# dendisuhubdy/neural_sound_generation

Hardware: AMD Instinct MI355X
Metric: mel-frames/sec VQ-VAE fwd+bwd+Adam (80-mel x 1024) (higher is better)
Workload: dtype bf16; 1 GPU; BASELINE configs[1]: VQVAE(1,dim=128,z_dim=512) train step, 128 clips/GPU x 80-mel x 1024 frames; clips_per_gpu=128, global_batch=128, frames=1024, parallelism=dp1

## Files before the change

neural_sound_generation_amd/csrc/gemm_patch.hip:

```cpp
#include "nsg_common.h"
#include <type_traits>

namespace {

NSG_DIAG_SWITCH(int, g_patch_gemm, 1)
NSG_DIAG_SWITCH(int, g_patch_grid_cap, 512)


inline int patch_grid(int ntiles, int ntn)
{
    const int cap = g_patch_grid_cap > 0 ? (g_patch_grid_cap / ntn > 0 ? g_patch_grid_cap / ntn : 1) : 0;
    return (cap > 0 && ntiles > cap) ? cap : ntiles;
}

constexpr int PG_MAX_JOBS = 16;
constexpr int PG_MAX_TAPS = 64;
constexpr int SLOT_BYTES = 16;

struct PatchJob {
    int c0_bytes;
    short jy, jx;
    short oy, ox;
    int flush;
};
struct PatchTap {
    int delta_bytes;
    unsigned woff_bytes;
};

struct PatchGemmParams {
    const bf16_t *in;
    const bf16_t *w;
    const float *bias;
    bf16_t *out;
    const bf16_t *epi_add;
    const bf16_t *epi_mask;
    int B, IH, IW, CI, OH, OW, CO;
    int tiles_y, tiles_x, ntiles;
    FastDiv div_tx, div_tyx;
    int njobs, ntaps;
    int sy, sx;
    int os;
    int flags;
    unsigned in_bytes, w_bytes;
    unsigned long long *stamps;
    float *stats;
    PatchJob jobs[PG_MAX_JOBS];
    PatchTap taps[PG_MAX_TAPS];
};

template <int PH, int PW, int NT, bool ADD, bool MASK, bool STAMP = false, bool STATS = false>
__global__ __launch_bounds__(256) __attribute__((amdgpu_waves_per_eu(2))) void patch_gemm_kernel(const PatchGemmParams p)
{
    constexpr bool PRIV = !(ADD || MASK);
    constexpr int NSLOT = PH * PW;
    constexpr int NPIECE = NSLOT * 8;
    constexpr int NP = (NPIECE + 255) / 256;
    constexpr int NB = (NT == 9) ? 3 : 4;
    constexpr int LD = (NT == 9) ? 3 : 2;
    static_assert(NT % NB == 0 && NB % LD == 0 && NB >= 2, "static buffer roles inside a body of NB taps");
    constexpr int NLOAD = NT - LD;
    constexpr int PPT = (NP + NLOAD - 1) / NLOAD;
    constexpr int NSLOT_PAD = (NSLOT + 15) / 16 * 16;
    constexpr int PLANE = NSLOT_PAD * 16;
    constexpr int BUF_BYTES = 8 * PLANE;
    constexpr int CPITCH = 132;
    static_assert(32 * CPITCH * 4 <= BUF_BYTES, "a tile row of the output must fit a retired patch buffer");
    static_assert(PPT * NLOAD >= NP && NT >= 4, "every patch piece is fetched LD taps before the job ends");
    constexpr unsigned OOB = 0xfffffff0u;

    constexpr int STG_PITCH = 36;
    constexpr int STG_BYTES = 32 * STG_PITCH * 4;

    extern __shared__ __attribute__((aligned(16))) char smem[];

    unsigned long long st_entry = 0, st_rt = 0, st_loop = 0, st_bound = 0, st_flush = 0, st_pro = 0, st_jobs = 0, st_t = 0;
    auto now = [&]() -> unsigned long long {
        if constexpr (STAMP) {
            unsigned long long t;
            __builtin_amdgcn_sched_barrier(0);
            asm volatile("s_memtime %0\n\ts_waitcnt lgkmcnt(0)" : "=s"(t) :: "memory");
            __builtin_amdgcn_sched_barrier(0);
            return t;
        }
        return 0ull;
    };
    if constexpr (STAMP) { st_entry = now(); st_rt = __builtin_amdgcn_s_memrealtime(); }

    const int tid = threadIdx.x;
    const int lane = tid & 63;
    const int wave = __builtin_amdgcn_readfirstlane(tid >> 6);
    const int x31 = lane & 31, h = lane >> 5;
    const int n0 = blockIdx.y * 128;

    const __amdgpu_buffer_rsrc_t rs_in = __builtin_amdgcn_make_buffer_rsrc(const_cast<bf16_t *>(p.in), 0, (int)p.in_bytes, 0x00020000);
    const __amdgpu_buffer_rsrc_t rs_w = __builtin_amdgcn_make_buffer_rsrc(const_cast<bf16_t *>(p.w), 0, (int)p.w_bytes, 0x00020000);

    const int slot0 = (tid & 7) + 8 * (tid >> 6);
    const unsigned piece_b = ((tid >> 3) & 7) * 16;
    const unsigned pc_lds0 = ((tid >> 3) & 7) * PLANE + slot0 * 16;

    const unsigned wlane = (unsigned)((((n0 >> 5) + wave) * 4 * 64 + lane) * 16);
    unsigned arow[4];
#pragma unroll
    for (int y = 0; y < 4; ++y) arow[y] = (unsigned)((y * PW + x31) * 16 + h * PLANE);

    const int cg = tid & 15;
    const int ep = lane >> 2, eq = lane & 3;
    const int ech = PRIV ? 32 * wave + 8 * eq : 8 * cg;
    float bv[8];
#pragma unroll
    for (int e = 0; e < 8; ++e) bv[e] = p.bias ? p.bias[n0 + ech + e] : 0.f;
    const bool relu_out = (p.flags & NSG_RELU_OUT) != 0;
    static_assert(!STATS || (PRIV && !ADD && !MASK), "statistics ride in the plain variant's wave-private epilogue");
    float st_sum[STATS ? 8 : 1], st_sq[STATS ? 8 : 1], st_pv[STATS ? 8 : 1], st_cnt = 0.f;
#pragma unroll
    for (int e = 0; e < (STATS ? 8 : 1); ++e) { st_sum[e] = 0.f; st_sq[e] = 0.f; st_pv[e] = 0.f; }

    const int tab_delta = p.taps[lane].delta_bytes;
    const int tab_woff = (int)p.taps[lane].woff_bytes;
    static_assert(PG_MAX_TAPS <= 64, "one lane per table entry");
    auto tap_delta = [&](int q) { return __builtin_amdgcn_readlane(tab_delta, q); };
    auto tap_woff = [&](int q) { return __builtin_amdgcn_readlane(tab_woff, q); };
    const PatchJob myjob = p.jobs[lane & (PG_MAX_JOBS - 1)];
    const int tabj_c0 = myjob.c0_bytes;
    const int tabj_j = ((int)myjob.jy & 0xffff) | ((int)myjob.jx << 16);
    const int tabj_o = (int)myjob.oy | ((int)myjob.ox << 8) | (myjob.flush << 16);
    auto job_entry = [&](int j) {
        const int c0 = __builtin_amdgcn_readlane(tabj_c0, j), jj = __builtin_amdgcn_readlane(tabj_j, j), oo = __builtin_amdgcn_readlane(tabj_o, j);
        return PatchJob{c0, (short)(jj & 0xffff), (short)(jj >> 16), (short)(oo & 0xff), (short)((oo >> 8) & 0xff), (oo >> 16) & 1};
    };

    v16f acc[4];
    v4f breg[NB][4];
    v4f afr[4];
    v4f ptmp[LD][PPT];

    const int G = gridDim.x;
    struct Cursor { int tile, job; };
    auto advance = [&](Cursor &c) {
        if (++c.job == p.njobs) { c.job = 0; c.tile += G; }
    };
    auto tile_origin = [&](int tile, int &b, int &ty, int &tx) {
        b = nsg_div(tile, p.div_tyx);
        const int rem = tile - b * (p.tiles_y * p.tiles_x);
        ty = nsg_div(rem, p.div_tx);
        tx = rem - ty * p.tiles_x;
    };

    int pt_ok = 0, pt_iy0 = 0, pt_ix0 = 0;
    unsigned pt_base = 0;
    auto patch_origin = [&](const Cursor &c) {
        pt_ok = c.tile < p.ntiles;
        int b, ty, tx;
        tile_origin(pt_ok ? c.tile : 0, b, ty, tx);
        const PatchJob jb = job_entry(c.job);
        pt_iy0 = ty * 4 * p.sy + jb.jy;
        pt_ix0 = tx * 32 * p.sx + jb.jx;
        pt_base = (unsigned)(b * p.IH * p.IW) * (unsigned)p.CI * 2u + (unsigned)jb.c0_bytes;
    };
    auto load_piece = [&](int r) -> v4f {
        const int slot = slot0 + 32 * r;
        const int yy = slot / PW, xx = slot - yy * PW;
        const int iy = pt_iy0 + yy * p.sy, ix = pt_ix0 + xx * p.sx;
        const bool ok = (slot < NSLOT) & (iy >= 0) & (iy < p.IH) & (ix >= 0) & (ix < p.IW) & (pt_ok != 0);
        const unsigned off = ok ? pt_base + (unsigned)((iy * p.IW + ix) * p.CI) * 2u + piece_b : OOB;
        return __builtin_bit_cast(v4f, __builtin_amdgcn_raw_buffer_load_b128(rs_in, (int)off, 0, 0));
    };
    auto store_piece = [&](int buf, int r, const v4f v) {
        if (slot0 + 32 * r < NSLOT) *reinterpret_cast<v4f *>(smem + buf * BUF_BYTES + pc_lds0 + r * 32 * 16) = v;
    };
    auto patch_traffic = [&](auto HALF, int t, int buf) __attribute__((always_inline)) {
        constexpr int hf = decltype(HALF)::value;
        if (t >= LD) {
#pragma unroll
            for (int i = 0; i < PPT; ++i)
                if ((t - LD) * PPT + i < NP) store_piece(buf ^ 1, (t - LD) * PPT + i, ptmp[hf][i]);
        }
        if (t < NLOAD) {
#pragma unroll
            for (int i = 0; i < PPT; ++i)
                if (t * PPT + i < NP) ptmp[hf][i] = load_piece(t * PPT + i);
        }
    };

    auto load_b = [&](v4f (&bq)[4], int q) {
        const int so = tap_woff(q);
#if defined(NSG_DIAG) && defined(NSG_PATCH_FAKEW)
        bq[0] = __builtin_bit_cast(v4f, __builtin_amdgcn_raw_buffer_load_b128(rs_w, (int)wlane, so, 0));
        bq[1] = bq[0]; bq[2] = bq[0]; bq[3] = bq[0];
        return;
#endif
#pragma unroll
        for (int kk = 0; kk < 4; ++kk)
            bq[kk] = __builtin_bit_cast(v4f, __builtin_amdgcn_raw_buffer_load_b128(rs_w, (int)(wlane + 1024 * kk), so, 0));
    };
    auto read_a = [&](int y, int buf, int q, int kk) {
        afr[y] = *reinterpret_cast<const v4f *>(smem + buf * BUF_BYTES + tap_delta(q) + 2 * kk * PLANE + arow[y]);
    };
    auto read_a_first = [&](int buf, int q) {
#pragma unroll
        for (int y = 0; y < 4; ++y) read_a(y, buf, q, 0);
    };
    auto mfma_chain = [&](const v4f (&bq)[4], int buf, int q, int qn) __attribute__((always_inline)) {
#pragma unroll
        for (int kk = 0; kk < 4; ++kk) {
#pragma unroll
            for (int y = 0; y < 4; ++y) {
                acc[y] = __builtin_amdgcn_mfma_f32_32x32x16_bf16(__builtin_bit_cast(bf16x8, bq[kk]), __builtin_bit_cast(bf16x8, afr[y]), acc[y], 0, 0, 0);
                if (kk < 3) read_a(y, buf, q, kk + 1);
                else read_a(y, buf, qn, 0);
            }
#pragma unroll
            for (int y = 0; y < 4; ++y) {
                __builtin_amdgcn_sched_group_barrier(0x008, 1, 0);
                __builtin_amdgcn_sched_group_barrier(0x100, 1, 0);
            }
        }
    };
    const unsigned out_bytes = (unsigned)(p.B * p.OH * p.OW) * (unsigned)p.CO * 2u;
    const __amdgpu_buffer_rsrc_t rs_out = __builtin_amdgcn_make_buffer_rsrc(p.out, 0, (int)out_bytes, 0x00020000);
    const __amdgpu_buffer_rsrc_t rs_add = __builtin_amdgcn_make_buffer_rsrc(const_cast<bf16_t *>(ADD ? p.epi_add : p.out), 0, (int)out_bytes, 0x00020000);
    const __amdgpu_buffer_rsrc_t rs_mask = __builtin_amdgcn_make_buffer_rsrc(const_cast<bf16_t *>(MASK ? p.epi_mask : p.out), 0, (int)out_bytes, 0x00020000);
    unsigned eoff[4][2];
    v4f addv[ADD ? 4 : 1][2], maskv[MASK ? 4 : 1][2];
    auto epi_offsets = [&](int tile, const PatchJob &jb, bool live) {
        int b, ty, tx;
        tile_origin(tile, b, ty, tx);
#pragma unroll
        for (int y = 0; y < 4; ++y)
#pragma unroll
            for (int e2 = 0; e2 < 2; ++e2) {
                const int oy = (ty * 4 + y) * p.os + jb.oy;
                const int ox = (tx * 32 + (PRIV ? ep : (tid >> 4)) + 16 * e2) * p.os + jb.ox;
                eoff[y][e2] = (live && oy < p.OH && ox < p.OW) ? (unsigned)(((b * p.OH + oy) * p.OW + ox) * p.CO + n0 + ech) * 2u : OOB;
            }
    };
    auto epi_prefetch = [&]() {
        if constexpr (ADD) {
#pragma unroll
            for (int y = 0; y < 4; ++y)
#pragma unroll
                for (int e2 = 0; e2 < 2; ++e2) addv[y][e2] = __builtin_bit_cast(v4f, __builtin_amdgcn_raw_buffer_load_b128(rs_add, (int)eoff[y][e2], 0, 0));
        }
        if constexpr (MASK) {
#pragma unroll
            for (int y = 0; y < 4; ++y)
#pragma unroll
                for (int e2 = 0; e2 < 2; ++e2) maskv[y][e2] = __builtin_bit_cast(v4f, __builtin_amdgcn_raw_buffer_load_b128(rs_mask, (int)eoff[y][e2], 0, 0));
        }
    };
    auto tap = [&](auto JJ, int buf, int t, int q, int qn, int qb) __attribute__((always_inline)) {
        constexpr int J = decltype(JJ)::value;
        const v4f (&bq)[4] = breg[J];
        load_b(breg[(J + NB - 1) % NB], qb);
        __builtin_amdgcn_sched_barrier(0);
        patch_traffic(std::integral_constant<int, J % LD>{}, t, buf);
        __builtin_amdgcn_sched_barrier(0);
        mfma_chain(bq, buf, q, qn);
    };
    auto zero_acc = [&]() {
#pragma unroll
        for (int y = 0; y < 4; ++y)
#pragma unroll
            for (int r = 0; r < 16; ++r) acc[y][r] = 0.f;
    };

    auto epi_piece = [&](const v4f t0, const v4f t1, int y, int e2) __attribute__((always_inline)) {
        float v[8] = {t0.x, t0.y, t0.z, t0.w, t1.x, t1.y, t1.z, t1.w};
#pragma unroll
        for (int e = 0; e < 8; ++e) v[e] += bv[e];
#pragma unroll
        for (int e = 0; e < 8; ++e) v[e] = relu_out ? fmaxf(v[e], 0.f) : v[e];
        if constexpr (ADD) {
            float t[8];
            Elem<bf16_t>::unpack16(addv[y][e2], t);
#pragma unroll
            for (int e = 0; e < 8; ++e) v[e] += t[e];
        }
        if constexpr (MASK) {
            float t[8];
            Elem<bf16_t>::unpack16(maskv[y][e2], t);
#pragma unroll
            for (int e = 0; e < 8; ++e) v[e] = t[e] > 0.f ? v[e] : 0.f;
        }
        unsigned u[4];
#pragma unroll
        for (int i = 0; i < 4; ++i) u[i] = nsg_pack_bf16(v[2 * i], v[2 * i + 1]);
        if constexpr (STATS) {
            const float live = eoff[y][e2] != OOB ? 1.f : 0.f;
#pragma unroll
            for (int i = 0; i < 4; ++i) {
                const float y0 = nsg_bitsf(u[i] << 16), y1 = nsg_bitsf(u[i] & 0xffff0000u);
                st_pv[2 * i] = (st_cnt == 0.f) ? y0 : st_pv[2 * i];
                st_pv[2 * i + 1] = (st_cnt == 0.f) ? y1 : st_pv[2 * i + 1];
                const float d0 = (y0 - st_pv[2 * i]) * live, d1 = (y1 - st_pv[2 * i + 1]) * live;
                st_sum[2 * i] += d0;
                st_sum[2 * i + 1] += d1;
                st_sq[2 * i] = __builtin_fmaf(d0, d0, st_sq[2 * i]);
                st_sq[2 * i + 1] = __builtin_fmaf(d1, d1, st_sq[2 * i + 1]);
            }
            st_cnt += live;
        }
        typedef unsigned u4 __attribute__((ext_vector_type(4)));
        __builtin_amdgcn_raw_buffer_store_b128(u4{u[0], u[1], u[2], u[3]}, rs_out, (int)eoff[y][e2], 0, 0);
    };
    auto flush = [&](int tile, const PatchJob &jb, int buf) __attribute__((always_inline)) {
        if constexpr (PRIV) {
            epi_offsets(tile, jb, true);
            float *Sw = reinterpret_cast<float *>(smem + 2 * BUF_BYTES + wave * STG_BYTES);
            float *wdst = Sw + x31 * STG_PITCH + 4 * h;
            const float *rsrc = Sw + ep * STG_PITCH + 8 * eq;
            auto put_row = [&](int y) {
#pragma unroll
                for (int g = 0; g < 4; ++g)
                    *reinterpret_cast<v4f *>(wdst + 8 * g) = v4f{acc[y][4 * g], acc[y][4 * g + 1], acc[y][4 * g + 2], acc[y][4 * g + 3]};
                __builtin_amdgcn_wave_barrier();
            };
            v4f rd[2][2][2];
            auto get_row = [&](int y) {
#pragma unroll
                for (int e2 = 0; e2 < 2; ++e2) {
                    rd[y & 1][e2][0] = *reinterpret_cast<const v4f *>(rsrc + 16 * e2 * STG_PITCH);
                    rd[y & 1][e2][1] = *reinterpret_cast<const v4f *>(rsrc + 16 * e2 * STG_PITCH + 4);
                }
                __builtin_amdgcn_wave_barrier();
            };
            put_row(0);
            get_row(0);
#pragma unroll
            for (int y = 0; y < 4; ++y) {
                if (y < 3) { put_row(y + 1); get_row(y + 1); }
#pragma unroll
                for (int e2 = 0; e2 < 2; ++e2) epi_piece(rd[y & 1][e2][0], rd[y & 1][e2][1], y, e2);
            }
            return;
        }
        epi_offsets(tile, jb, true);
        epi_prefetch();
        float *Cs = reinterpret_cast<float *>(smem + buf * BUF_BYTES);
#pragma unroll
        for (int y = 0; y < 4; ++y) {
#pragma unroll
            for (int g = 0; g < 4; ++g) {
                float *dst = Cs + x31 * CPITCH + 32 * wave + 8 * g + 4 * h;
                *reinterpret_cast<v4f *>(dst) = v4f{acc[y][4 * g], acc[y][4 * g + 1], acc[y][4 * g + 2], acc[y][4 * g + 3]};
            }
            __syncthreads();
#pragma unroll
            for (int e2 = 0; e2 < 2; ++e2) {
                const int px = (tid >> 4) + 16 * e2;
                epi_piece(*reinterpret_cast<const v4f *>(Cs + px * CPITCH + 8 * cg), *reinterpret_cast<const v4f *>(Cs + px * CPITCH + 8 * cg + 4), y, e2);
            }
            __syncthreads();
        }
    };

    int bid = blockIdx.x;
    {
        const int xcd = bid & 7, qq = G >> 3, rr = G & 7;
        bid = (xcd < rr ? xcd * (qq + 1) : rr * (qq + 1) + (xcd - rr) * qq) + (bid >> 3);
    }
    Cursor cur = {bid, 0};
    Cursor pre = cur;
    if (cur.tile >= p.ntiles) return;
    patch_origin(pre);
    for (int r = 0; r < NP; ++r) store_piece(0, r, load_piece(r));
#pragma unroll
    for (int j = 0; j + 1 < NB; ++j) load_b(breg[j], j);
    zero_acc();
    __syncthreads();
    int buf = 0;
    auto run_job = [&](int qbase, int qnext_base) __attribute__((always_inline)) {
        using NO = std::integral_constant<bool, false>;
        using YES = std::integral_constant<bool, true>;
        auto tq = [&](int t) { return t < NT ? qbase + t : qnext_base + (t - NT); };
        auto body = [&](int t0, auto LASTBODY) __attribute__((always_inline)) {
            constexpr bool LB = decltype(LASTBODY)::value;
#define NSG_TAP(J)                                                                                                              \
            if constexpr (J < NB) {                                                                                             \
                constexpr int NEXT = (LB && J == NB - 1) ? 0 : 1;                                                               \
                tap(std::integral_constant<int, J>{}, buf, t0 + J, qbase + t0 + J, qbase + t0 + J + NEXT, tq(t0 + J + NB - 1)); \
            }
            NSG_TAP(0) NSG_TAP(1) NSG_TAP(2) NSG_TAP(3)
#undef NSG_TAP
        };
        read_a_first(buf, qbase);
#pragma unroll 1
        for (int t0 = 0; t0 < NT - NB; t0 += NB) body(t0, NO{});
        body(NT - NB, YES{});
    };
    if constexpr (STAMP) st_pro = now() - st_entry;
    auto do_job = [&]() __attribute__((always_inline)) {
        if constexpr (STAMP) st_t = now();
        const PatchJob jb = job_entry(cur.job);
        advance(pre);
        patch_origin(pre);
        const int qbase = cur.job * NT;
        const int qnext = (cur.job + 1 == p.njobs ? 0 : cur.job + 1) * NT;
        run_job(qbase, qnext);
        if constexpr (STAMP) { const unsigned long long t = now(); st_loop += t - st_t; st_t = t; st_jobs += 1; }
        __syncthreads();
        if constexpr (STAMP) { const unsigned long long t = now(); st_bound += t - st_t; st_t = t; }
        if (jb.flush) {
            flush(cur.tile, jb, buf);
            zero_acc();
            if constexpr (STAMP) { const unsigned long long t = now(); st_flush += t - st_t; st_t = t; }
        }
        advance(cur);
        buf ^= 1;
    };
    for (;;) {
        if (cur.tile >= p.ntiles) break;
        do_job();
    }
    if constexpr (STATS) {
        __syncthreads();
        float *red = reinterpret_cast<float *>(smem);
        const float inv = st_cnt > 0.f ? 1.f / st_cnt : 0.f;
#pragma unroll
        for (int e = 0; e < 8; ++e) {
            red[e * 256 + tid] = st_pv[e] + st_sum[e] * inv;
            red[(8 + e) * 256 + tid] = fmaxf(st_sq[e] - st_sum[e] * st_sum[e] * inv, 0.f);
        }
        red[16 * 256 + tid] = st_cnt;
        __syncthreads();
        if (tid < 128) {
            const int ch = tid, wv = ch >> 5, eqq = (ch >> 3) & 3, e = ch & 7;
            double N = 0.0, S = 0.0;
            for (int r = 0; r < 16; ++r) {
                const int t = wv * 64 + r * 4 + eqq;
                const double n = red[16 * 256 + t];
                N += n;
                S += n * (double)red[e * 256 + t];
            }
            const double mu = N > 0.0 ? S / N : 0.0;
            double Q = 0.0;
            for (int r = 0; r < 16; ++r) {
                const int t = wv * 64 + r * 4 + eqq;
                const double n = red[16 * 256 + t];
                const double dl = (double)red[e * 256 + t] - mu;
                Q += n > 0.0 ? (double)red[(8 + e) * 256 + t] + n * dl * dl : 0.0;
            }
            float *dst = p.stats + (size_t)blockIdx.x * 3 * p.CO + n0 + ch;
            dst[0] = (float)N;
            dst[p.CO] = (float)S;
            dst[2 * p.CO] = (float)Q;
        }
    }
    if constexpr (STAMP) {
        if (tid == 0 && p.stamps) {
            unsigned long long *o = p.stamps + 8 * (size_t)(blockIdx.y * gridDim.x + blockIdx.x);
            o[0] = now() - st_entry; o[1] = __builtin_amdgcn_s_memrealtime() - st_rt; o[2] = st_loop; o[3] = st_bound;
            o[4] = st_flush; o[5] = st_pro; o[6] = st_jobs;
#ifdef NSG_PATCH_ABS_STAMPS
            o[3] = st_rt; o[5] = __builtin_amdgcn_s_memrealtime();
#endif
            o[7] = ((unsigned long long)__builtin_amdgcn_s_getreg(6164) << 32) | (unsigned)__builtin_amdgcn_s_getreg(63492);
        }
    }
}

template <int PH, int PW, int NT, bool ADD, bool MASK, bool STAMP, bool STATS = false>
int launch_patch(const PatchGemmParams &p, int ntiles_n, hipStream_t s)
{
    constexpr int NSLOT = PH * PW;
    constexpr size_t BUF_BYTES = (size_t)8 * ((NSLOT + 15) / 16 * 16) * 16;
    constexpr bool PRIV = !(ADD || MASK);
    const size_t lds = 2 * BUF_BYTES + (PRIV ? 4 * 32 * 36 * 4 : 0);
    static LdsOptIn once;
    if (lds > 65536) {
        const int rc = nsg_lds_opt_in(once, {reinterpret_cast<const void *>(&patch_gemm_kernel<PH, PW, NT, ADD, MASK, STAMP, STATS>)}, lds, "patch_gemm");
        if (rc != NSG_OK) return rc;
    }
    const int gx = patch_grid(p.ntiles, ntiles_n);
    hipLaunchKernelGGL((patch_gemm_kernel<PH, PW, NT, ADD, MASK, STAMP, STATS>), dim3((unsigned)gx, (unsigned)ntiles_n), dim3(256), lds, s, p);
    return nsg_check_launch("patch_gemm");
}

template <int PH, int PW, int NT, bool STAMP>
int launch_patch_epi(const PatchGemmParams &p, int ntiles_n, hipStream_t s)
{
    if constexpr (!STAMP) {
        if (p.stats) return launch_patch<PH, PW, NT, false, false, false, true>(p, ntiles_n, s);
    }
    if (p.epi_add && p.epi_mask) return launch_patch<PH, PW, NT, true, true, STAMP>(p, ntiles_n, s);
    if (p.epi_add) return launch_patch<PH, PW, NT, true, false, STAMP>(p, ntiles_n, s);
    if (p.epi_mask) return launch_patch<PH, PW, NT, false, true, STAMP>(p, ntiles_n, s);
    return launch_patch<PH, PW, NT, false, false, STAMP>(p, ntiles_n, s);
}


}

#ifdef NSG_DIAG
extern "C" NSG_API void nsg_debug_set_patch_gemm(int on) { g_patch_gemm = on; }
extern "C" NSG_API void nsg_debug_set_patch_grid(int cap) { g_patch_grid_cap = cap; }
#endif

static int patch_kind(const GatherGemmParams &g)
{
    if (!g_patch_gemm) return -1;
    if (g.in_dtype != NSG_BF16 || g.out_dtype != NSG_BF16) return -1;
    if (g.flags & (NSG_RELU_IN | NSG_TANH_OUT)) return -1;
    if (g.stats && (g.epi_add || g.epi_mask || (g.flags & NSG_RELU_OUT) || g.stamps)) return -1;
    if (g.CI % 64 != 0 || g.CO % 128 != 0) return -1;
    const int chunks = g.CI / 64;
    int kind;
    if (g.mode == 1) kind = 2;
    else if (g.KH == 3 && g.KW == 3 && g.stride == 1 && g.pad >= 0 && g.pad <= 2 && g.pad_w >= 0 && g.pad_w <= 2) kind = 0;
    else if (g.KH == 4 && g.KW == 4 && g.stride == 2 && g.pad == 1 && g.pad_w == 1) kind = 1;
    else return -1;
    const int njobs = kind == 0 ? chunks : 4 * chunks;
    const int ntaps = kind == 0 ? 9 : 4;
    if (njobs > PG_MAX_JOBS || njobs * ntaps > PG_MAX_TAPS) return -1;
    if ((int64_t)g.B * nsg_cdiv(g.RH, 4) * nsg_cdiv(g.RW, 32) > 0x3fffffff) return -1;
    return kind;
}

int nsg_patch_gemm_stat_records(const GatherGemmParams &g)
{
    if (patch_kind(g) < 0) return 0;
    return patch_grid((int)((int64_t)g.B * nsg_cdiv(g.RH, 4) * nsg_cdiv(g.RW, 32)), g.CO / 128);
}

int nsg_launch_patch_gemm(const GatherGemmParams &g, hipStream_t s, bool *handled)
{
    *handled = false;
    const int kind = patch_kind(g);
    if (kind < 0) return NSG_OK;
    const int chunks = g.CI / 64;
    const int njobs = kind == 0 ? chunks : 4 * chunks;
    const int ntaps = kind == 0 ? 9 : 4;

    PatchGemmParams p = {};
    p.in = reinterpret_cast<const bf16_t *>(g.in);
    const int64_t wtaps = g.mode == 0 ? g.KH * g.KW : 16;
    const int64_t image = wtaps * g.CO * g.CI;
    p.w = reinterpret_cast<const bf16_t *>(g.w) + image;
    p.bias = g.bias;
    p.out = reinterpret_cast<bf16_t *>(g.out);
    p.epi_add = reinterpret_cast<const bf16_t *>(g.epi_add);
    p.epi_mask = reinterpret_cast<const bf16_t *>(g.epi_mask);
    p.B = g.B; p.IH = g.IH; p.IW = g.IW; p.CI = g.CI; p.OH = g.OH; p.OW = g.OW; p.CO = g.CO;
    constexpr int tcols = 32;
    constexpr int pw3 = tcols + 2, pw2 = tcols + 1;
    p.tiles_y = (int)nsg_cdiv(g.RH, 4);
    p.tiles_x = (int)nsg_cdiv(g.RW, tcols);
    const int64_t nt = (int64_t)g.B * p.tiles_y * p.tiles_x;
    if (nt > 0x3fffffff) return NSG_OK;
    p.ntiles = (int)nt;
    p.div_tx = nsg_fastdiv((uint32_t)p.tiles_x);
    p.div_tyx = nsg_fastdiv((uint32_t)p.tiles_y * (uint32_t)p.tiles_x);
    p.njobs = njobs; p.ntaps = ntaps;
    p.sy = p.sx = kind == 1 ? 2 : 1;
    p.os = kind == 2 ? 2 : 1;
    p.flags = g.flags;
    p.in_bytes = g.in_bytes; p.w_bytes = g.w_bytes;
    p.stamps = g.stamps;
    p.stats = g.stats;
    const int64_t blk = (int64_t)(g.CO / 32) * 4096;
    auto wblock = [&](int ws, int c) { return (unsigned)(((int64_t)ws * chunks + c) * blk); };
    int j = 0;
    if (kind == 0) {
        for (int c = 0; c < chunks; ++c, ++j) {
            p.jobs[j] = PatchJob{c * 128, (short)-g.pad, (short)-g.pad_w, 0, 0, c + 1 == chunks};
            for (int kh = 0; kh < 3; ++kh)
                for (int kw = 0; kw < 3; ++kw)
                    p.taps[j * 9 + kh * 3 + kw] = PatchTap{(kh * pw3 + kw) * SLOT_BYTES, wblock(kh * 3 + kw, c)};
        }
    } else if (kind == 1) {
        for (int c = 0; c < chunks; ++c)
            for (int pl = 0; pl < 4; ++pl, ++j) {
                const int ph = pl >> 1, pw = pl & 1;
                p.jobs[j] = PatchJob{c * 128, (short)(ph - 1), (short)(pw - 1), 0, 0, j + 1 == njobs};
                for (int a = 0; a < 2; ++a)
                    for (int b = 0; b < 2; ++b)
                        p.taps[j * 4 + a * 2 + b] = PatchTap{(a * pw2 + b) * SLOT_BYTES,
                                                           wblock((2 * a + ph) * 4 + (2 * b + pw), c)};
            }
    } else {
        for (int cls = 0; cls < 4; ++cls) {
            const int py = cls >> 1, px = cls & 1;
            for (int c = 0; c < chunks; ++c, ++j) {
                p.jobs[j] = PatchJob{c * 128, (short)(py - 1), (short)(px - 1), (short)py, (short)px, c + 1 == chunks};
                for (int a = 0; a < 2; ++a)
                    for (int b = 0; b < 2; ++b)
                        p.taps[j * 4 + a * 2 + b] = PatchTap{((1 - a) * pw2 + (1 - b)) * SLOT_BYTES,
                                                           wblock(((1 - py) + 2 * a) * 4 + (1 - px) + 2 * b, c)};
            }
        }
    }
    *handled = true;
    const int ntn = g.CO / 128;
#ifdef NSG_DIAG
    if (g.stamps) {
        if (kind == 0) return launch_patch_epi<6, 34, 9, true>(p, ntn, s);
        return launch_patch_epi<5, 33, 4, true>(p, ntn, s);
    }
#endif
    if (kind == 0) return launch_patch_epi<6, 34, 9, false>(p, ntn, s);
    return launch_patch_epi<5, 33, 4, false>(p, ntn, s);
}
```

Measured before the change: 16.32 million mel-frames/s.

## Add 512-thread LDS-staged patch GEMM with 64-column tiles and weight ring

```diff
diff --git a/neural_sound_generation_amd/csrc/gemm_patch.hip b/neural_sound_generation_amd/csrc/gemm_patch.hip
--- a/neural_sound_generation_amd/csrc/gemm_patch.hip
+++ b/neural_sound_generation_amd/csrc/gemm_patch.hip
@@ -7,9 +7,10 @@
 NSG_DIAG_SWITCH(int, g_patch_grid_cap, 512)
 
 
-inline int patch_grid(int ntiles, int ntn)
+inline int patch_grid(int ntiles, int ntn, int per_cu)
 {
-    const int cap = g_patch_grid_cap > 0 ? (g_patch_grid_cap / ntn > 0 ? g_patch_grid_cap / ntn : 1) : 0;
+    const int slots = g_patch_grid_cap * per_cu / 2;
+    const int cap = slots > 0 ? (slots / ntn > 0 ? slots / ntn : 1) : 0;
     return (cap > 0 && ntiles > cap) ? cap : ntiles;
 }
 
@@ -473,7 +474,7 @@
         const int rc = nsg_lds_opt_in(once, {reinterpret_cast<const void *>(&patch_gemm_kernel<PH, PW, NT, ADD, MASK, STAMP, STATS>)}, lds, "patch_gemm");
         if (rc != NSG_OK) return rc;
     }
-    const int gx = patch_grid(p.ntiles, ntiles_n);
+    const int gx = patch_grid(p.ntiles, ntiles_n, 2);
     hipLaunchKernelGGL((patch_gemm_kernel<PH, PW, NT, ADD, MASK, STAMP, STATS>), dim3((unsigned)gx, (unsigned)ntiles_n), dim3(256), lds, s, p);
     return nsg_check_launch("patch_gemm");
 }
@@ -488,6 +489,410 @@
     if (p.epi_add) return launch_patch<PH, PW, NT, true, false, STAMP>(p, ntiles_n, s);
     if (p.epi_mask) return launch_patch<PH, PW, NT, false, true, STAMP>(p, ntiles_n, s);
     return launch_patch<PH, PW, NT, false, false, STAMP>(p, ntiles_n, s);
+}
+
+template <int KIND, bool ADD, bool MASK, bool STATS = false>
+__global__ __launch_bounds__(512) __attribute__((amdgpu_waves_per_eu(2))) void patch_gemm_lds_kernel(const PatchGemmParams p)
+{
+    constexpr bool PRIV = !(ADD || MASK);
+    constexpr int NT = KIND == 0 ? 9 : 4;
+    constexpr int PH = KIND == 0 ? 6 : 5;
+    constexpr int PW = KIND == 0 ? 66 : 65;
+    constexpr int NSLOT = PH * PW;
+    constexpr int NGRP = (NSLOT + 7) / 8;
+    constexpr int NRND = (NGRP + 7) / 8;
+    constexpr int PBUF = NRND * 8 * 1024;
+    constexpr int R = NT % 3 == 0 ? 3 : 4;
+    constexpr int WBLK = 16384;
+    constexpr int RING0 = 2 * PBUF;
+    constexpr int NLT = NT - 2;
+    constexpr int PPT = (NRND + NLT - 1) / NLT;
+    static_assert(NT % R == 0 && R >= 3, "static ring roles: a job starts at ring block 0; refill three taps ahead");
+    static_assert(RING0 + R * WBLK <= 163840, "LDS");
+    static_assert(PBUF <= 65536, "patch buffer 1 is addressed by the ds_read offset field");
+    constexpr int CPITCH = 132;
+    constexpr int STG_PITCH = 36;
+    constexpr int STG_BYTES = 32 * STG_PITCH * 4;
+    static_assert(64 * CPITCH * 4 <= PBUF && 8 * STG_BYTES <= PBUF && 17 * 512 * 4 <= PBUF, "epilogue staging fits a retired patch buffer");
+    constexpr unsigned OOB = 0xfffffff0u;
+    typedef __attribute__((address_space(3))) void *lds_ptr_t;
+
+    extern __shared__ __attribute__((aligned(16))) char smem_l[];
+    char *const smem = smem_l;
+
+    const int tid = threadIdx.x;
+    const int lane = tid & 63;
+    const int wave = __builtin_amdgcn_readfirstlane(tid >> 6);
+    const int ph = wave >> 2, cq = wave & 3;
+    const int x31 = lane & 31, h = lane >> 5;
+    const int n0 = blockIdx.y * 128;
+
+    const __amdgpu_buffer_rsrc_t rs_in = __builtin_amdgcn_make_buffer_rsrc(const_cast<bf16_t *>(p.in), 0, (int)p.in_bytes, 0x00020000);
+    const __amdgpu_buffer_rsrc_t rs_w = __builtin_amdgcn_make_buffer_rsrc(const_cast<bf16_t *>(p.w), 0, (int)p.w_bytes, 0x00020000);
+
+    auto tap_delta = [](int t) constexpr -> int {
+        if (KIND == 0) return (t / 3) * PW + t % 3;
+        if (KIND == 1) return (t >> 1) * PW + (t & 1);
+        return (1 - (t >> 1)) * PW + (1 - (t & 1));
+    };
+    unsigned fa[4][NT];
+#pragma unroll
+    for (int y = 0; y < 4; ++y)
+#pragma unroll
+        for (int t = 0; t < NT; ++t) {
+            const unsigned s = (unsigned)(y * PW + 32 * ph + x31 + tap_delta(t));
+            fa[y][t] = s * 128u + 16u * ((unsigned)h ^ ((s >> 1) & 7u));
+        }
+    const unsigned wl = (unsigned)(RING0 + cq * 4096 + lane * 16);
+
+    const int tab_woff = (int)p.taps[lane].woff_bytes;
+    static_assert(PG_MAX_TAPS <= 64, "one lane per table entry");
+    auto tap_woff = [&](int q) { return __builtin_amdgcn_readlane(tab_woff, q); };
+    const PatchJob myjob = p.jobs[lane & (PG_MAX_JOBS - 1)];
+    const int tabj_c0 = myjob.c0_bytes;
+    const int tabj_j = ((int)myjob.jy & 0xffff) | ((int)myjob.jx << 16);
+    const int tabj_o = (int)myjob.oy | ((int)myjob.ox << 8) | (myjob.flush << 16);
+    auto job_entry = [&](int j) {
+        const int c0 = __builtin_amdgcn_readlane(tabj_c0, j), jj = __builtin_amdgcn_readlane(tabj_j, j), oo = __builtin_amdgcn_readlane(tabj_o, j);
+        return PatchJob{c0, (short)(jj & 0xffff), (short)(jj >> 16), (short)(oo & 0xff), (short)((oo >> 8) & 0xff), (oo >> 16) & 1};
+    };
+
+    const int cg = tid & 15;
+    const int ep = lane >> 2, eq = lane & 3;
+    const int ech = PRIV ? 32 * cq + 8 * eq : 8 * cg;
+    float bv[8];
+#pragma unroll
+    for (int e = 0; e < 8; ++e) bv[e] = p.bias ? p.bias[n0 + ech + e] : 0.f;
+    const bool relu_out = (p.flags & NSG_RELU_OUT) != 0;
+    static_assert(!STATS || PRIV, "statistics ride in the plain variant's wave-private epilogue");
+    float st_sum[STATS ? 8 : 1], st_sq[STATS ? 8 : 1], st_pv[STATS ? 8 : 1], st_cnt = 0.f;
+#pragma unroll
+    for (int e = 0; e < (STATS ? 8 : 1); ++e) { st_sum[e] = 0.f; st_sq[e] = 0.f; st_pv[e] = 0.f; }
+
+    v16f acc[4];
+    v4f bq[2][4];
+    v4f afr[4];
+
+    const int G = gridDim.x;
+    struct Cursor { int tile, job; };
+    auto advance = [&](Cursor &c) {
+        if (++c.job == p.njobs) { c.job = 0; c.tile += G; }
+    };
+    auto tile_origin = [&](int tile, int &b, int &ty, int &tx) {
+        b = nsg_div(tile, p.div_tyx);
+        const int rem = tile - b * (p.tiles_y * p.tiles_x);
+        ty = nsg_div(rem, p.div_tx);
+        tx = rem - ty * p.tiles_x;
+    };
+
+    int pt_ok = 0, pt_iy0 = 0, pt_ix0 = 0;
+    unsigned pt_base = 0;
+    auto patch_origin = [&](const Cursor &c) {
+        pt_ok = c.tile < p.ntiles;
+        int b, ty, tx;
+        tile_origin(pt_ok ? c.tile : 0, b, ty, tx);
+        const PatchJob jb = job_entry(c.job);
+        pt_iy0 = ty * 4 * p.sy + jb.jy;
+        pt_ix0 = tx * 64 * p.sx + jb.jx;
+        pt_base = (unsigned)(b * p.IH * p.IW) * (unsigned)p.CI * 2u + (unsigned)jb.c0_bytes;
+    };
+    const int lslot = lane >> 3, lpiece = lane & 7;
+    auto dma_patch = [&](int buf, int r) {
+        const int g = 8 * r + wave;
+        const int slot = 8 * g + lslot;
+        const int yy = slot / PW, xx = slot - yy * PW;
+        const int iy = pt_iy0 + yy * p.sy, ix = pt_ix0 + xx * p.sx;
+        const bool ok = (slot < NSLOT) & (iy >= 0) & (iy < p.IH) & (ix >= 0) & (ix < p.IW) & (pt_ok != 0);
+        const unsigned piece = (unsigned)(lpiece ^ ((slot >> 1) & 7));
+        const unsigned off = ok ? pt_base + (unsigned)((iy * p.IW + ix) * p.CI) * 2u + piece * 16u : OOB;
+        __builtin_amdgcn_raw_ptr_buffer_load_lds(rs_in, (lds_ptr_t)(smem + buf * PBUF + g * 1024), 16, (int)off, 0, 0, 0);
+    };
+    const unsigned wsrc = (unsigned)((n0 >> 5) * 4096 + wave * 1024 + lane * 16);
+    auto dma_w = [&](int k, int q) {
+        const int so = tap_woff(q);
+#pragma unroll
+        for (int i = 0; i < 2; ++i)
+            __builtin_amdgcn_raw_ptr_buffer_load_lds(rs_w, (lds_ptr_t)(smem + RING0 + k * WBLK + i * 8192 + wave * 1024), 16,
+                                                     (int)(wsrc + i * 8192), so, 0, 0);
+    };
+    auto read_w = [&](v4f (&bw)[4], int k, int kk) {
+        bw[kk] = *reinterpret_cast<const v4f *>(smem + wl + k * WBLK + kk * 1024);
+    };
+    constexpr bool LEAN = ADD || MASK || STATS;
+    auto read_a = [&](int y, int buf, int t, int kk) {
+        unsigned a = fa[y][t];
+        if constexpr (LEAN) asm("" : "+v"(a));
+        afr[y] = *reinterpret_cast<const v4f *>(smem + buf * PBUF + (a ^ (unsigned)(32 * kk)));
+    };
+    auto zero_acc = [&]() {
+#pragma unroll
+        for (int y = 0; y < 4; ++y)
+#pragma unroll
+            for (int r = 0; r < 16; ++r) acc[y][r] = 0.f;
+    };
+
+    const unsigned out_bytes = (unsigned)(p.B * p.OH * p.OW) * (unsigned)p.CO * 2u;
+    const __amdgpu_buffer_rsrc_t rs_out = __builtin_amdgcn_make_buffer_rsrc(p.out, 0, (int)out_bytes, 0x00020000);
+    const __amdgpu_buffer_rsrc_t rs_add = __builtin_amdgcn_make_buffer_rsrc(const_cast<bf16_t *>(ADD ? p.epi_add : p.out), 0, (int)out_bytes, 0x00020000);
+    const __amdgpu_buffer_rsrc_t rs_mask = __builtin_amdgcn_make_buffer_rsrc(const_cast<bf16_t *>(MASK ? p.epi_mask : p.out), 0, (int)out_bytes, 0x00020000);
+    unsigned eoff[4][2];
+    v4f addv[ADD ? 4 : 1][2], maskv[MASK ? 4 : 1][2];
+    auto epi_offsets = [&](int tile, const PatchJob &jb) {
+        int b, ty, tx;
+        tile_origin(tile, b, ty, tx);
+#pragma unroll
+        for (int y = 0; y < 4; ++y)
+#pragma unroll
+            for (int e2 = 0; e2 < 2; ++e2) {
+                const int oy = (ty * 4 + y) * p.os + jb.oy;
+                const int ox = (tx * 64 + (PRIV ? 32 * ph + ep + 16 * e2 : (tid >> 4) + 32 * e2)) * p.os + jb.ox;
+                eoff[y][e2] = (oy < p.OH && ox < p.OW) ? (unsigned)(((b * p.OH + oy) * p.OW + ox) * p.CO + n0 + ech) * 2u : OOB;
+            }
+    };
+    auto epi_piece = [&](const v4f t0, const v4f t1, int y, int e2) __attribute__((always_inline)) {
+        float v[8] = {t0.x, t0.y, t0.z, t0.w, t1.x, t1.y, t1.z, t1.w};
+#pragma unroll
+        for (int e = 0; e < 8; ++e) v[e] += bv[e];
+#pragma unroll
+        for (int e = 0; e < 8; ++e) v[e] = relu_out ? fmaxf(v[e], 0.f) : v[e];
+        if constexpr (ADD) {
+            float t[8];
+            Elem<bf16_t>::unpack16(addv[y][e2], t);
+#pragma unroll
+            for (int e = 0; e < 8; ++e) v[e] += t[e];
+        }
+        if constexpr (MASK) {
+            float t[8];
+            Elem<bf16_t>::unpack16(maskv[y][e2], t);
+#pragma unroll
+            for (int e = 0; e < 8; ++e) v[e] = t[e] > 0.f ? v[e] : 0.f;
+        }
+        unsigned u[4];
+#pragma unroll
+        for (int i = 0; i < 4; ++i) u[i] = nsg_pack_bf16(v[2 * i], v[2 * i + 1]);
+        if constexpr (STATS) {
+            const float live = eoff[y][e2] != OOB ? 1.f : 0.f;
+#pragma unroll
+            for (int i = 0; i < 4; ++i) {
+                const float y0 = nsg_bitsf(u[i] << 16), y1 = nsg_bitsf(u[i] & 0xffff0000u);
+                st_pv[2 * i] = (st_cnt == 0.f) ? y0 : st_pv[2 * i];
+                st_pv[2 * i + 1] = (st_cnt == 0.f) ? y1 : st_pv[2 * i + 1];
+                const float d0 = (y0 - st_pv[2 * i]) * live, d1 = (y1 - st_pv[2 * i + 1]) * live;
+                st_sum[2 * i] += d0;
+                st_sum[2 * i + 1] += d1;
+                st_sq[2 * i] = __builtin_fmaf(d0, d0, st_sq[2 * i]);
+                st_sq[2 * i + 1] = __builtin_fmaf(d1, d1, st_sq[2 * i + 1]);
+            }
+            st_cnt += live;
+        }
+        typedef unsigned u4 __attribute__((ext_vector_type(4)));
+        __builtin_amdgcn_raw_buffer_store_b128(u4{u[0], u[1], u[2], u[3]}, rs_out, (int)eoff[y][e2], 0, 0);
+    };
+    auto lds_barrier = [&]() {
+        __builtin_amdgcn_sched_barrier(0);
+        asm volatile("s_waitcnt lgkmcnt(0)\n\ts_barrier" ::: "memory");
+        __builtin_amdgcn_sched_barrier(0);
+    };
+    constexpr int EPI_VMEM = 8;
+    auto flush = [&](int tile, const PatchJob &jb, int buf) __attribute__((always_inline)) {
+        epi_offsets(tile, jb);
+        if constexpr (PRIV) {
+            float *Sw = reinterpret_cast<float *>(smem + buf * PBUF + wave * STG_BYTES);
+            float *wdst = Sw + x31 * STG_PITCH + 4 * h;
+            const float *rsrc = Sw + ep * STG_PITCH + 8 * eq;
+            auto put_row = [&](int y) {
+#pragma unroll
+                for (int g = 0; g < 4; ++g)
+                    *reinterpret_cast<v4f *>(wdst + 8 * g) = v4f{acc[y][4 * g], acc[y][4 * g + 1], acc[y][4 * g + 2], acc[y][4 * g + 3]};
+                __builtin_amdgcn_wave_barrier();
+            };
+            v4f rd[2][2][2];
+            auto get_row = [&](int y) {
+#pragma unroll
+                for (int e2 = 0; e2 < 2; ++e2) {
+                    rd[y & 1][e2][0] = *reinterpret_cast<const v4f *>(rsrc + 16 * e2 * STG_PITCH);
+                    rd[y & 1][e2][1] = *reinterpret_cast<const v4f *>(rsrc + 16 * e2 * STG_PITCH + 4);
+                }
+                __builtin_amdgcn_wave_barrier();
+            };
+            put_row(0);
+            get_row(0);
+#pragma unroll
+            for (int y = 0; y < 4; ++y) {
+                if (y < 3) { put_row(y + 1); get_row(y + 1); }
+#pragma unroll
+                for (int e2 = 0; e2 < 2; ++e2) epi_piece(rd[y & 1][e2][0], rd[y & 1][e2][1], y, e2);
+            }
+            return;
+        }
+        if constexpr (ADD) {
+#pragma unroll
+            for (int y = 0; y < 4; ++y)
+#pragma unroll
+                for (int e2 = 0; e2 < 2; ++e2) addv[y][e2] = __builtin_bit_cast(v4f, __builtin_amdgcn_raw_buffer_load_b128(rs_add, (int)eoff[y][e2], 0, 0));
+        }
+        if constexpr (MASK) {
+#pragma unroll
+            for (int y = 0; y < 4; ++y)
+#pragma unroll
+                for (int e2 = 0; e2 < 2; ++e2) maskv[y][e2] = __builtin_bit_cast(v4f, __builtin_amdgcn_raw_buffer_load_b128(rs_mask, (int)eoff[y][e2], 0, 0));
+        }
+        float *Cs = reinterpret_cast<float *>(smem + buf * PBUF);
+#pragma unroll
+        for (int y = 0; y < 4; ++y) {
+#pragma unroll
+            for (int g = 0; g < 4; ++g) {
+                float *dst = Cs + (32 * ph + x31) * CPITCH + 32 * cq + 8 * g + 4 * h;
+                *reinterpret_cast<v4f *>(dst) = v4f{acc[y][4 * g], acc[y][4 * g + 1], acc[y][4 * g + 2], acc[y][4 * g + 3]};
+            }
+            lds_barrier();
+#pragma unroll
+            for (int e2 = 0; e2 < 2; ++e2) {
+                const int px = (tid >> 4) + 32 * e2;
+                epi_piece(*reinterpret_cast<const v4f *>(Cs + px * CPITCH + 8 * cg), *reinterpret_cast<const v4f *>(Cs + px * CPITCH + 8 * cg + 4), y, e2);
+            }
+            lds_barrier();
+        }
+    };
+
+    int bid = blockIdx.x;
+    {
+        const int xcd = bid & 7, qq = G >> 3, rr = G & 7;
+        bid = (xcd < rr ? xcd * (qq + 1) : rr * (qq + 1) + (xcd - rr) * qq) + (bid >> 3);
+    }
+    Cursor cur = {bid, 0};
+    if (cur.tile >= p.ntiles) return;
+    patch_origin(cur);
+#pragma unroll
+    for (int r = 0; r < NRND; ++r) dma_patch(0, r);
+#pragma unroll
+    for (int t = 0; t < 3; ++t) dma_w(t, t);
+    zero_acc();
+    __builtin_amdgcn_sched_barrier(0);
+    asm volatile("s_waitcnt vmcnt(2)" ::: "memory");
+    lds_barrier();
+#pragma unroll
+    for (int kk = 0; kk < 4; ++kk) read_w(bq[0], 0, kk);
+#pragma unroll
+    for (int y = 0; y < 4; ++y) read_a(y, 0, 0, 0);
+
+    bool flushed = false;
+    auto do_job = [&](auto BUF) __attribute__((always_inline)) {
+        constexpr int buf = decltype(BUF)::value;
+        const PatchJob jb = job_entry(cur.job);
+        const int jn = cur.job + 1 == p.njobs ? 0 : cur.job + 1;
+        Cursor pre = cur;
+        advance(pre);
+        patch_origin(pre);
+        const int qb = cur.job * NT, qn = jn * NT;
+        auto tap = [&](auto TT) __attribute__((always_inline)) {
+            constexpr int t = decltype(TT)::value;
+            constexpr int cb = (buf * NT + t) & 1;
+            if constexpr (t >= 1 && t <= NT - 2) {
+#pragma unroll
+                for (int i = 0; i < PPT; ++i)
+                    if ((t - 1) * PPT + i < NRND) dma_patch(buf ^ 1, (t - 1) * PPT + i);
+            }
+            dma_w((t + 3) % R, t + 3 < NT ? qb + t + 3 : qn + t + 3 - NT);
+            __builtin_amdgcn_sched_barrier(0);
+#pragma unroll
+            for (int kk = 0; kk < 4; ++kk) {
+#pragma unroll
+                for (int y = 0; y < 4; ++y) {
+                    acc[y] = __builtin_amdgcn_mfma_f32_32x32x16_bf16(__builtin_bit_cast(bf16x8, bq[cb][kk]), __builtin_bit_cast(bf16x8, afr[y]), acc[y], 0, 0, 0);
+                    if (kk < 3) read_a(y, buf, t, kk + 1);
+                    else if (t + 1 < NT) read_a(y, buf, t + 1, 0);
+                    else read_a(y, buf ^ 1, 0, 0);
+                    if (kk == 1) read_w(bq[cb ^ 1], (t + 1) % R, y);
+                }
+#pragma unroll
+                for (int y = 0; y < 4; ++y) {
+                    __builtin_amdgcn_sched_group_barrier(0x008, 1, 0);
+                    if (kk == 1) __builtin_amdgcn_sched_group_barrier(0x100, 2, 0);
+                    else __builtin_amdgcn_sched_group_barrier(0x100, 1, 0);
+                }
+            }
+            constexpr int pieces = (t >= 1 && t < NT - 2) ? (NRND - (t - 1) * PPT < PPT ? NRND - (t - 1) * PPT : PPT) : 0;
+            static_assert(pieces >= 0, "");
+            __builtin_amdgcn_sched_barrier(0);
+            if (t == 0 && flushed) asm volatile("s_waitcnt vmcnt(%0)" :: "n"(2 + EPI_VMEM) : "memory");
+            else asm volatile("s_waitcnt vmcnt(%0)" :: "n"(2 + pieces) : "memory");
+            lds_barrier();
+        };
+#define NSG_TAP(T) if constexpr (T < NT) tap(std::integral_constant<int, T>{});
+        NSG_TAP(0) NSG_TAP(1) NSG_TAP(2) NSG_TAP(3) NSG_TAP(4) NSG_TAP(5) NSG_TAP(6) NSG_TAP(7) NSG_TAP(8)
+#undef NSG_TAP
+        static_assert(NT <= 9, "");
+        flushed = jb.flush != 0;
+        if (jb.flush) {
+            flush(cur.tile, jb, buf);
+            zero_acc();
+        }
+        advance(cur);
+    };
+    for (;;) {
+        do_job(std::integral_constant<int, 0>{});
+        if (cur.tile >= p.ntiles) break;
+        do_job(std::integral_constant<int, 1>{});
+        if (cur.tile >= p.ntiles) break;
+    }
+    asm volatile("s_waitcnt vmcnt(0)" ::: "memory");
+    if constexpr (STATS) {
+        __syncthreads();
+        float *red = reinterpret_cast<float *>(smem);
+        const float inv = st_cnt > 0.f ? 1.f / st_cnt : 0.f;
+#pragma unroll
+        for (int e = 0; e < 8; ++e) {
+            red[e * 512 + tid] = st_pv[e] + st_sum[e] * inv;
+            red[(8 + e) * 512 + tid] = fmaxf(st_sq[e] - st_sum[e] * st_sum[e] * inv, 0.f);
+        }
+        red[16 * 512 + tid] = st_cnt;
+        __syncthreads();
+        if (tid < 128) {
+            const int ch = tid, wv = ch >> 5, eqq = (ch >> 3) & 3, e = ch & 7;
+            double N = 0.0, S = 0.0;
+            for (int r = 0; r < 32; ++r) {
+                const int t = ((r >> 4) * 4 + wv) * 64 + (r & 15) * 4 + eqq;
+                const double n = red[16 * 512 + t];
+                N += n;
+                S += n * (double)red[e * 512 + t];
+            }
+            const double mu = N > 0.0 ? S / N : 0.0;
+            double Q = 0.0;
+            for (int r = 0; r < 32; ++r) {
+                const int t = ((r >> 4) * 4 + wv) * 64 + (r & 15) * 4 + eqq;
+                const double n = red[16 * 512 + t];
+                const double dl = (double)red[e * 512 + t] - mu;
+                Q += n > 0.0 ? (double)red[(8 + e) * 512 + t] + n * dl * dl : 0.0;
+            }
+            float *dst = p.stats + (size_t)blockIdx.x * 3 * p.CO + n0 + ch;
+            dst[0] = (float)N;
+            dst[p.CO] = (float)S;
+            dst[2 * p.CO] = (float)Q;
+        }
+    }
+}
+
+template <int KIND, bool ADD, bool MASK, bool STATS = false>
+int launch_patch_lds(const PatchGemmParams &p, int ntiles_n, hipStream_t s)
+{
+    constexpr size_t lds = 163840;
+    static LdsOptIn once;
+    const int rc = nsg_lds_opt_in(once, {reinterpret_cast<const void *>(&patch_gemm_lds_kernel<KIND, ADD, MASK, STATS>)}, lds, "patch_gemm");
+    if (rc != NSG_OK) return rc;
+    const int gx = patch_grid(p.ntiles, ntiles_n, 1);
+    hipLaunchKernelGGL((patch_gemm_lds_kernel<KIND, ADD, MASK, STATS>), dim3((unsigned)gx, (unsigned)ntiles_n), dim3(512), lds, s, p);
+    return nsg_check_launch("patch_gemm");
+}
+
+template <int KIND>
+int launch_patch_lds_epi(const PatchGemmParams &p, int ntiles_n, hipStream_t s)
+{
+    if (p.stats) return launch_patch_lds<KIND, false, false, true>(p, ntiles_n, s);
+    if (p.epi_add && p.epi_mask) return launch_patch_lds<KIND, true, true>(p, ntiles_n, s);
+    if (p.epi_add) return launch_patch_lds<KIND, true, false>(p, ntiles_n, s);
+    if (p.epi_mask) return launch_patch_lds<KIND, false, true>(p, ntiles_n, s);
+    return launch_patch_lds<KIND, false, false>(p, ntiles_n, s);
 }
 
 
@@ -518,10 +923,18 @@
     return kind;
 }
 
+static bool patch_use_lds(const GatherGemmParams &g, int kind)
+{
+    if (g_patch_gemm == 2) return false;
+    if (g_patch_gemm == 3) return true;
+    return kind != 2 && !g.epi_add && !g.epi_mask && !g.stats;
+}
+
 int nsg_patch_gemm_stat_records(const GatherGemmParams &g)
 {
     if (patch_kind(g) < 0) return 0;
-    return patch_grid((int)((int64_t)g.B * nsg_cdiv(g.RH, 4) * nsg_cdiv(g.RW, 32)), g.CO / 128);
+    const int tcols = patch_use_lds(g, patch_kind(g)) ? 64 : 32;
+    return patch_grid((int)((int64_t)g.B * nsg_cdiv(g.RH, 4) * nsg_cdiv(g.RW, tcols)), g.CO / 128, tcols == 64 ? 1 : 2);
 }
 
 int nsg_launch_patch_gemm(const GatherGemmParams &g, hipStream_t s, bool *handled)
@@ -543,8 +956,9 @@
     p.epi_add = reinterpret_cast<const bf16_t *>(g.epi_add);
     p.epi_mask = reinterpret_cast<const bf16_t *>(g.epi_mask);
     p.B = g.B; p.IH = g.IH; p.IW = g.IW; p.CI = g.CI; p.OH = g.OH; p.OW = g.OW; p.CO = g.CO;
-    constexpr int tcols = 32;
-    constexpr int pw3 = tcols + 2, pw2 = tcols + 1;
+    const bool lds = patch_use_lds(g, kind);
+    const int tcols = lds ? 64 : 32;
+    const int pw3 = tcols + 2, pw2 = tcols + 1;
     p.tiles_y = (int)nsg_cdiv(g.RH, 4);
     p.tiles_x = (int)nsg_cdiv(g.RW, tcols);
     const int64_t nt = (int64_t)g.B * p.tiles_y * p.tiles_x;
@@ -593,6 +1007,11 @@
     }
     *handled = true;
     const int ntn = g.CO / 128;
+    if (lds) {
+        if (kind == 0) return launch_patch_lds_epi<0>(p, ntn, s);
+        if (kind == 1) return launch_patch_lds_epi<1>(p, ntn, s);
+        return launch_patch_lds_epi<2>(p, ntn, s);
+    }
 #ifdef NSG_DIAG
     if (g.stamps) {
         if (kind == 0) return launch_patch_epi<6, 34, 9, true>(p, ntn, s);
```

Result: no change. 16.41 million mel-frames/s (median of 6 runs) (+0.5%).
